# smacke/ffsubsync

Measured on AMD Instinct MI355X. Metric: alignments/sec (2 h@100 Hz, 7 framerate ratios), higher is better.
Workload: dtype i32; 1 GPU; configs[2]: 8192 x 7200 s@100 Hz pairs per GPU (8 batches of 1024), MaxScoreAligner over 7 framerate ratios, max_offset_samples=6000; algorithm=auto, pairs_per_gpu=8192, pairs_in_flight=512, n_fft_reference=2097152, n_fft_device=786432, input_format=bit-packed 0/1 vectors (FFS_DTYPE_U1) resident in HBM, parallelism=single GPU

## Files before the change

ffsubsync_amd/csrc/ffs_runs.h:

```cpp
#pragma once
#include "ffs_kernels.h"

namespace ffsa {

#ifndef FFS_RUNS_THREADS
#define FFS_RUNS_THREADS 512
#define FFS_RUNS_T 12288
#define FFS_RUNS_QCAP 3070
#endif
constexpr int RUNS_THREADS = FFS_RUNS_THREADS;
constexpr int RUNS_WAVES = RUNS_THREADS / 64;
constexpr int RUNS_T = FFS_RUNS_T;
constexpr int RUNS_LPT = RUNS_T / RUNS_THREADS;
constexpr int RUNS_QCAP = FFS_RUNS_QCAP;
static_assert(RUNS_T % RUNS_THREADS == 0 && RUNS_LPT % 4 == 0 && RUNS_LPT <= 32, "whole groups of four lags per thread, 32-bit edge windows");
constexpr int RUNS_CAP = 32768;
#ifndef FFS_RUNS_TPW
#define FFS_RUNS_TPW 2
#endif
constexpr int RUNS_TPW = FFS_RUNS_TPW;
constexpr int RUNS_QSENT = 0x1fffffff;
static_assert(RUNS_LPT <= 32 && RUNS_LPT % 4 == 0 && RUNS_QCAP % 2 == 0, "one 32-bit mask per thread, 8-byte histogram loads");

struct RunsRef {
// ... 67 lines not shown
}

FFS_DEV float wave_max_f32(float v) {
#define FFS_DPP_MAX(ctrl, rows) v = fmaxf(v, __int_as_float(__builtin_amdgcn_update_dpp(__float_as_int(v), __float_as_int(v), ctrl, rows, 0xf, false)))
    FFS_DPP_MAX(0x111, 0xf);
    FFS_DPP_MAX(0x112, 0xf);
    FFS_DPP_MAX(0x114, 0xf);
    FFS_DPP_MAX(0x118, 0xf);
    FFS_DPP_MAX(0x142, 0xa);
    FFS_DPP_MAX(0x143, 0xc);
#undef FFS_DPP_MAX
    return __int_as_float(__builtin_amdgcn_readlane(__float_as_int(v), 63));
}

constexpr int RUNS_XQ = 256;
template <int NT>
FFS_DEV void runs_extract_lds(unsigned (*&s_e)[NT / 64 * 2], unsigned (*&s_o)[NT / 64 * 2], uint4 (*&s_q)[RUNS_XQ]) {
    __shared__ unsigned l_e[2][NT / 64 * 2], l_o[2][NT / 64 * 2];
    __shared__ __attribute__((aligned(16))) uint4 l_q[NT / 64][RUNS_XQ];
    s_e = l_e, s_o = l_o, s_q = l_q;
}
template <int NT, bool compact = false>
FFS_DEV void runs_extract_body(const unsigned* __restrict__ w_generic, const int len, int2* __restrict__ e, int2* __restrict__ hdr,
                               const int cap) {
    constexpr int NWV = NT / 64;
    constexpr int G = 2, SWEEP = NT * 4 * G;
    const int tid = threadIdx.x, lane = tid & 63, wave = __builtin_amdgcn_readfirstlane(tid >> 6);
    const gptr eb = (gptr)e;
    const int nw = (len + 31) >> 5;
    const int n_proc = (len >> 5) + 1;
    const unsigned tail = (len & 31) ? ((1u << (len & 31)) - 1u) : 0xffffffffu;
    unsigned(*s_e)[NWV * 2], (*s_o)[NWV * 2];
    uint4(*s_q)[RUNS_XQ];
    runs_extract_lds<NT>(s_e, s_o, s_q);
    uint4* const ring = s_q[wave];
    unsigned q_head = 0, q_tail = 0;
    unsigned n_bound = 0, n_ones = 0;
    unsigned xn[G][4], pn[G];
    const __amdgpu_buffer_rsrc_t vrs = __builtin_amdgcn_make_buffer_rsrc(const_cast<unsigned*>(w_generic), 0, nw * 4, 0x00020000);
    auto request = [&](int base) {
#pragma unroll
        for (int g = 0; g < G; ++g) {
            const int w0 = base + (g * NT + tid) * 4;
            typedef unsigned v4u __attribute__((ext_vector_type(4)));
            const v4u t = __builtin_amdgcn_raw_buffer_load_b128(vrs, w0 * 4, 0, 2);
            xn[g][0] = t.x, xn[g][1] = t.y, xn[g][2] = t.z, xn[g][3] = t.w;
            pn[g] = 0;
            if (lane == 0) pn[g] = __builtin_amdgcn_raw_buffer_load_b32(vrs, w0 * 4 - 4, 0, 0);
        }
    };
// ... 162 lines not shown
        long long est = (long long)cnt * (long long)r.len / sampled;
        if (est > 0x3fffffff) est = 0x3fffffff;
        const_cast<int2*>(r.hdr)[0] = make_int2((int)est, 0);
    }
}

FFS_DEV void runs_extract_zero(int* __restrict__ zero, int zero_words) {
    if (zero && blockIdx.x == 0)
        for (int i = threadIdx.x; i < zero_words; i += blockDim.x) zero[i] = 0;
}
FFS_DEV bool runs_compact_vec(int cstride, int n_plain) {
    return cstride > 0 && (int)blockIdx.x < n_plain && (int)blockIdx.x % cstride != 0;
}
__global__ __launch_bounds__(256, 8) void k_runs_extract(const RunsRef* __restrict__ refs, int* __restrict__ zero, int zero_words,
                                                         int cstride, int n_plain) {
    runs_extract_zero(zero, zero_words);
    const RunsRef r = refs[blockIdx.x];
    if (!r.bits) return;
    if (runs_compact_vec(cstride, n_plain))
        runs_extract_body<256, true>(r.bits, r.len, const_cast<int2*>(r.e), const_cast<int2*>(r.hdr), r.cap);
    else
        runs_extract_body<256, false>(r.bits, r.len, const_cast<int2*>(r.e), const_cast<int2*>(r.hdr), r.cap);
}
__global__ __launch_bounds__(512, 4) void k_runs_extract_512(const RunsRef* __restrict__ refs, int with_len_cap, int* __restrict__ zero,
                                                             int zero_words, int cstride, int n_plain) {
    runs_extract_zero(zero, zero_words);
    const RunsRef r = refs[blockIdx.x];
    if (!r.bits) return;
    if (with_len_cap && threadIdx.x == 0) const_cast<int2*>(r.hdr)[1] = make_int2(r.len, r.cap);
    if (runs_compact_vec(cstride, n_plain))
        runs_extract_body<512, true>(r.bits, r.len, const_cast<int2*>(r.e), const_cast<int2*>(r.hdr), r.cap);
    else
        runs_extract_body<512, false>(r.bits, r.len, const_cast<int2*>(r.e), const_cast<int2*>(r.hdr), r.cap);
}
__global__ __launch_bounds__(1024, 4) void k_runs_extract_1024(const RunsRef* __restrict__ refs, int with_len_cap, int* __restrict__ zero,
                                                               int zero_words, int cstride, int n_plain) {
    runs_extract_zero(zero, zero_words);
    const RunsRef r = refs[blockIdx.x];
    if (!r.bits) return;
    if (with_len_cap && threadIdx.x == 0) const_cast<int2*>(r.hdr)[1] = make_int2(r.len, r.cap);
    if (runs_compact_vec(cstride, n_plain))
        runs_extract_body<1024, true>(r.bits, r.len, const_cast<int2*>(r.e), const_cast<int2*>(r.hdr), r.cap);
    else
        runs_extract_body<1024, false>(r.bits, r.len, const_cast<int2*>(r.e), const_cast<int2*>(r.hdr), r.cap);
}

__global__ __launch_bounds__(256, 8) void k_runs_extract_lists(const RunsRef* __restrict__ refs) {
    const RunsRef r = refs[blockIdx.x];
    if (threadIdx.x == 0) const_cast<int2*>(r.hdr)[1] = make_int2(r.len, r.cap);
    runs_extract_body<256>(r.bits, r.len, const_cast<int2*>(r.e), const_cast<int2*>(r.hdr), r.cap);
}

__global__ __launch_bounds__(1024, 4) void k_runs_extract_one(const unsigned* __restrict__ bits, int len, int2* __restrict__ e,
                                                             int2* __restrict__ hdr, int cap) {
    if (threadIdx.x == 0) hdr[1] = make_int2(len, cap);
    runs_extract_body<1024>(bits, len, e, hdr, cap);
}

static inline void runs_extract_launch(const RunsRef* refs, size_t n_vec, bool with_len_cap, hipStream_t st, int* zero = nullptr,
                                       int zero_words = 0, int cstride = 0, int n_plain = 0) {
    if (with_len_cap) cstride = 0;
    if (n_vec <= 256)
        hipLaunchKernelGGL(k_runs_extract_1024, dim3((unsigned)n_vec), dim3(1024), 0, st, refs, with_len_cap ? 1 : 0, zero, zero_words, cstride, n_plain);
    else if (n_vec <= 768)
        hipLaunchKernelGGL(k_runs_extract_512, dim3((unsigned)n_vec), dim3(512), 0, st, refs, with_len_cap ? 1 : 0, zero, zero_words, cstride, n_plain);
    else if (with_len_cap)
        hipLaunchKernelGGL(k_runs_extract_lists, dim3((unsigned)n_vec), dim3(256), 0, st, refs);
    else
        hipLaunchKernelGGL(k_runs_extract, dim3((unsigned)n_vec), dim3(256), 0, st, refs, zero, zero_words, cstride, n_plain);
}

FFS_DEV unsigned fetch32(GWords w, int len, long long start) {
    const int nw = (len + 31) >> 5;
    const long long wi = start >> 5;
    unsigned v[2];
#pragma unroll
    for (int k = 0; k < 2; ++k) {
        const long long i = wi + k;
        unsigned t = (i >= 0 && i < nw) ? w[i] : 0u;
        if (i == nw - 1 && (len & 31)) t &= (1u << (len & 31)) - 1u;
        v[k] = t;
    }
    return __builtin_amdgcn_alignbit(v[1], v[0], (unsigned)(start & 31));
}

FFS_DEV unsigned list_bits32(GEntries e, int n, long long start) {
    if (start + 32 <= 0 || n <= 0) return 0u;
    int lo = 0, hi = n;
    while (lo < hi) {
        const int mid = (lo + hi) >> 1;
        if ((long long)e[mid].pos <= start)
            lo = mid + 1;
// ... 1100 lines not shown
```

ffsubsync_amd/csrc/ffsalign.hip:

```cpp
#include <hip/hip_runtime.h>
#if defined(__x86_64__) && !defined(__HIP_DEVICE_COMPILE__)
#include <immintrin.h>
#define FFS_HOST_AVX2 1
#else
#define FFS_HOST_AVX2 0
#endif
#include <dlfcn.h>
#include <math.h>
#include <stdarg.h>
#include <stdio.h>
#include <stdlib.h>
#include <string.h>

#include <algorithm>
#include <chrono>
#include <string>
#include <mutex>
#include <vector>

#include "../../include/ffsubsync_amd.h"
#include "ffs_kernels.h"
#include "ffs_runs.h"
#include "ffs_split.h"
#include "ffs_quality.h"
// ... 52 lines not shown
            constexpr int DT = 4;                 \
            stmt;                                 \
        } else if ((dtype) == FFS_DTYPE_U8) {     \
            constexpr int DT = 0;                 \
            stmt;                                 \
        } else if ((dtype) == FFS_DTYPE_F32) {    \
            constexpr int DT = 1;                 \
            stmt;                                 \
        } else if ((dtype) == FFS_DTYPE_F64) {    \
            constexpr int DT = 3;                 \
            stmt;                                 \
        } else {                                  \
            constexpr int DT = 2;                 \
            stmt;                                 \
        }                                         \
    } while (0)

constexpr int64_t kMinFftN = 4096;
constexpr int64_t kMaxFftN = 1 << 24;
constexpr unsigned kPoolCapacity = 1u << 20;
constexpr long long kRunsBudgetPerPoint = 12;
constexpr int kRunsStride0 = 4096;
constexpr size_t kSmallCallCands = 4096;
constexpr int kSegBlocks = 3;
constexpr int kCollectRows = 4;

int ilog2(int64_t x) {
    int p = 0;
    while ((int64_t(1) << p) < x) ++p;
    return p;
}

int tile_cols(int L) {
    if (L % 3 == 0) {
        const int c = 3072 / L;
        return c < 16 ? 16 : c;
    }
    if (L <= 16) return 256;
    if (L <= 128) return 4096 / L;
    if (L <= 1024) return 16;
    if (L == 2048) return 8;
    return 4;
}

size_t col_lds_bytes(int L) {
    size_t t = (L > 16) ? (size_t)L * tile_cols(L) * sizeof(cf) : 0;
// ... 81 lines not shown
    int64_t workspace_bytes = 0;
    bool radix3_off = false;
    bool workspace_ready = false;
    int algo = FFS_ALGO_AUTO;
    int runs_split = 0;
    long long runs_budget = -1;
    int2* runs_e = nullptr;
    int runs_stride = 4096;
    size_t runs_e_entries = 0;
    int2* runs_n = nullptr;
    size_t runs_vecs = 0;
    unsigned* pack_buf = nullptr;
    size_t pack_bytes = 0;
    int* runs_flags = nullptr;
    int* runs_zero_flags = nullptr;
    int* runs_flags_host = nullptr;
    size_t runs_flags_n = 0;
    RunsBest* runs_best = nullptr;
    size_t runs_best_n = 0;
    bool runs_prev_fft = false;
    unsigned* lvl_buf = nullptr;
    size_t lvl_bytes = 0;
    hipEvent_t runs_ev = nullptr;
    int64_t runs_calls = 0, runs_fft_chunks = 0, runs_chunks = 0, runs_last_boundaries = 0;
    bool host_timing = false;
    double ht_vec = 0, ht_cand = 0, ht_wait = 0, ht_decide = 0, ht_total = 0;
    mutable std::vector<const void*> lds_configured;
    bool profiling = false;
    std::vector<hipEvent_t> ev_pool;
    size_t ev_used = 0;
    std::vector<std::pair<int, std::pair<hipEvent_t, hipEvent_t>>> ev_spans;
};

namespace {

template <class T>
int upload(T** dst, const std::vector<T>& src, int64_t* total) {
    HIP_TRY(hipMalloc((void**)dst, src.size() * sizeof(T)));
    HIP_TRY(hipMemcpy(*dst, src.data(), src.size() * sizeof(T), hipMemcpyHostToDevice));
    *total += (int64_t)(src.size() * sizeof(T));
    return FFS_OK;
}

int ensure_desc(ffs_plan* p, size_t bytes) {
    if (bytes <= p->dev_desc_bytes) return FFS_OK;
    if (p->upload_done) HIP_TRY(hipEventSynchronize(p->upload_done));
// ... 17 lines not shown
    static hipStream_t streams[64] = {};
    if (device < 0 || device >= 64) return nullptr;
    std::lock_guard<std::mutex> lock(mu);
    if (!streams[device] && hipStreamCreateWithFlags(&streams[device], hipStreamNonBlocking) != hipSuccess) {
        (void)hipGetLastError();
        streams[device] = nullptr;
    }
    return streams[device];
}
bool ensure_copy(ffs_plan* p) {
    if (!p->copy_stream) {
        p->copy_stream = shared_copy_stream(p->device);
        if (!p->copy_stream) return false;
    }
    if (!p->copy_ev && hipEventCreateWithFlags(&p->copy_ev, hipEventDisableTiming) != hipSuccess) {
        (void)hipGetLastError();
        p->copy_ev = nullptr;
        return false;
    }
    if (!p->dev_desc2 && hipMalloc(&p->dev_desc2, p->dev_desc_bytes) != hipSuccess) {
        (void)hipGetLastError();
        p->dev_desc2 = nullptr;
        return false;
    }
    return true;
}

int ensure_lds(const ffs_plan* p, const void* fn, size_t bytes) {
    for (const void* f : p->lds_configured)
        if (f == fn) return FFS_OK;
    HIP_TRY(hipFuncSetAttribute(fn, hipFuncAttributeMaxDynamicSharedMemorySize, (int)bytes));
    p->lds_configured.push_back(fn);
    return FFS_OK;
}

int ensure_workspace(ffs_plan* p) {
    if (p->direct_only || p->workspace_ready) return FFS_OK;
    const size_t work_bytes = (size_t)p->pairs_in_flight * p->max_slots * p->N * sizeof(cf);
    const size_t bn_bytes = (size_t)p->pairs_in_flight * (p->max_slots - 1) * 2 * (p->N2 / p->C) * sizeof(BlockNom);
    bool ok = hipMalloc((void**)&p->work, work_bytes) == hipSuccess;
    ok = ok && hipMalloc((void**)&p->bnom, bn_bytes) == hipSuccess;
    ok = ok && hipMalloc((void**)&p->xlist, (1 + (size_t)p->pairs_in_flight * p->max_cand) * sizeof(int)) == hipSuccess;
    ok = ok && hipMalloc((void**)&p->pool_entries, (size_t)kPoolCapacity * sizeof(PoolEntry)) == hipSuccess;
    int rc = FFS_OK;
    if (!ok) {
        (void)hipGetLastError();
// ... 662 lines not shown
    HIP_TRY(hipEventCreateWithFlags(&p->upload_done, hipEventDisableTiming));
    HIP_TRY(hipEventCreateWithFlags(&p->last_done, hipEventDisableTiming));
    for (int h = 0; h < 2; ++h) HIP_TRY(hipEventCreateWithFlags(&p->half_done[h], hipEventDisableTiming));
    {
        auto on = [](const char* name) {
            const char* e = getenv(name);
            return e && e[0] == '1';
        };
        p->allow_pruned = !on("FFS_DISABLE_PRUNED_PASS_C");
        p->allow_seg = !on("FFS_DISABLE_SEGMENTED");
        p->allow_half_last = !on("FFS_DISABLE_HALF_LAST");
        if (const char* ea = getenv("FFS_ALGORITHM")) {
            if (!strcmp(ea, "fft")) p->algo = FFS_ALGO_FFT;
            else if (!strcmp(ea, "runs")) p->algo = FFS_ALGO_RUNS;
        }
        p->runs_budget = -1;
        if (const char* eb = getenv("FFS_RUNS_BUDGET")) p->runs_budget = atoll(eb);
        if (const char* es = getenv("FFS_RUNS_SPLIT")) p->runs_split = atoi(es);
        p->runs_stride = kRunsStride0;
        if (const char* es = getenv("FFS_RUNS_STRIDE")) {
            const int v = atoi(es);
            p->runs_stride = v < 64 ? 64 : (v > RUNS_CAP ? RUNS_CAP : v);
        }
        if (const char* et = getenv("FFS_HOST_TIMING")) p->host_timing = et[0] == '1';
        const char* e3 = getenv("FFS_PASS_A_PREFETCH");
        if (e3) p->pass_a_prefetch = p->pass_a_prefetch_bits = atoi(e3);
#ifdef FFS_LAB
        const char* e20 = getenv("FFS_PASS_A_DEBUG");
        if (e20) p->lab_flags |= (atoi(e20) & 31) << 10;
        const char* e15 = getenv("FFS_MID_DEBUG");
        if (e15) p->lab_flags |= ((atoi(e15) & 1) ? DBG_NO_FFT : 0) | ((atoi(e15) & 2) ? DBG_HOT_MEM : 0) | ((atoi(e15) & 4) ? DBG_NO_STORE : 0);
#endif
    }
    if (n_fft < kMinFftN) {
        p->direct_only = true;
        guard.p = nullptr;
        *out = p;
        return FFS_OK;
    }
    if (r3) {
        p->N2 = n_fft >= 48 * 4096 ? 4096 : (int)(n_fft / 48);
        p->N1 = (int)(n_fft / p->N2);
    } else {
        const int lg = ilog2(n_fft);
        const int lg2 = lg - 4 < 12 ? lg - 4 : 12;
        p->N2 = 1 << lg2;
// ... 82 lines not shown
    (void)hipFree(p->tbA);
    (void)hipFree(p->tsA);
    (void)hipFree(p->tw1h);
    (void)hipFree(p->tbR);
    (void)hipFree(p->tsR);
    (void)hipFree(p->thR);
    (void)hipFree(p->tbM);
    (void)hipFree(p->tsM);
    (void)hipFree(p->twn1);
    (void)hipFree(p->work);
    (void)hipFree(p->bnom);
    (void)hipFree(p->pool_entries);
    (void)hipFree(p->xlist);
    if (p->seg) (void)ffs_plan_destroy(p->seg);
    (void)hipFree(p->runs_e);
    (void)hipFree(p->runs_n);
    (void)hipFree(p->runs_best);
    (void)hipFree(p->runs_flags);
    (void)hipFree(p->runs_zero_flags);
    (void)hipFree(p->pack_buf);
    (void)hipFree(p->lvl_buf);
    if (p->runs_flags_host) (void)hipHostFree(p->runs_flags_host);
    if (p->runs_ev) (void)hipEventDestroy(p->runs_ev);
    if (p->upload_done) (void)hipEventSynchronize(p->upload_done);
    if (p->copy_ev) (void)hipEventDestroy(p->copy_ev);
    for (int h = 0; h < 2; ++h)
        if (p->half_done[h]) (void)hipEventDestroy(p->half_done[h]);
    (void)hipFree(p->dev_desc);
    (void)hipFree(p->dev_desc2);
    if (p->host_desc) (void)hipHostFree(p->host_desc);
    if (p->upload_done) (void)hipEventDestroy(p->upload_done);
    if (p->last_done) (void)hipEventDestroy(p->last_done);
    for (hipEvent_t e : p->ev_pool) (void)hipEventDestroy(e);
    delete p;
    return FFS_OK;
}

int64_t ffs_plan_workspace_bytes(const ffs_plan* p) { return p ? p->workspace_bytes : 0; }

}

namespace {

struct AlignArgs {
    int n_pairs, n_cand, ref_dt, dtype;
    const void* const* vec_ptr;
// ... 183 lines not shown
    int32_t* level_lens(char* b) const { return (int32_t*)(b + o_ml); }
    int32_t* level_words(char* b) const { return (int32_t*)(b + o_mw); }
    XformDesc* xforms(char* b) const { return (XformDesc*)(b + o_xf); }
    NomList* nominees(char* b) const { return (NomList*)(b + o_nom); }
    RescoreAcc* acc(char* b) const { return (RescoreAcc*)(b + o_acc); }
    PoolBest* pool_best(char* b) const { return (PoolBest*)(b + o_pbest); }
    size_t table_at() const { return o_rv; }
    size_t table_bytes(size_t n_refs) const { return n_refs * sizeof(RunsRef); }
    size_t level_tables_bytes() const { return o_xf - o_rv; }
    size_t head_bytes(size_t n_refs) const { return o_rv + n_refs * sizeof(RunsRef); }
    size_t transform_bytes(size_t n_xf) const { return o_xf + n_xf * sizeof(XformDesc); }
    size_t refresh_at() const { return o_cand; }
    size_t refresh_bytes(size_t n_xf) const { return transform_bytes(n_xf) - o_cand; }
    size_t acc_bytes(size_t n) const { return n * KNOM * sizeof(RescoreAcc); }
    size_t acc_and_best_bytes() const { return acc_bytes(n_cands) + n_cands * sizeof(PoolBest); }
};

struct StreamLeave {
    ffs_plan* p;
    hipStream_t st;
    bool armed = false;
    bool upload_open = false;
    hipStream_t upload_st = nullptr;
    ~StreamLeave() {
        if (upload_open) (void)hipEventRecord(p->upload_done, upload_st);
        if (armed) (void)leave_stream(p, st);
    }
};

struct AlignCall {
    ffs_plan* const p;
    const AlignArgs& a;
    const hipStream_t st;
    StreamLeave leave;
    const int n_pairs, n_cand, stride, n_packed, n_slots, n_chunks;
    const size_t n_vec, n_cands;
    size_t n_rr = 0;
    size_t flag_bytes = 0;
    bool lists_in, ml, runs_ok, need_extract, ml_on = false, mixed, use_copy = false, dense_stream = false;
    int t_dtype, t_ref_dt;
    int hflags = 0;
    long long budget = 0;
    DescLayout L;
    char *hb = nullptr, *db = nullptr;
    CandDesc* hc = nullptr;
    const CandDesc* dc = nullptr;
    const RunsRef* d_rv = nullptr;
    const XformDesc* dx = nullptr;
    NomList* dn = nullptr;
    RescoreAcc* da = nullptr;
    PoolBest* dpb = nullptr;
    PoolArgs pa{};
    CandResult* cres;
    PairResult* pres;
    bool late_extract = false;
    bool probe_first = false;
    bool flags_cleared = false;
    bool copy_entered = false;
    bool proven = false, xf_built = false, retry = false;
    int tiles_max = 1;
    int64_t lvl_len_max = 1;
    const void* const* xptr;
    std::vector<const void*> expanded;
    BinList bins;
    bool pruned = false, seg = false;
    int seg_blocks = 0;
    int64_t seg_lo = 0;
    size_t n_xf;
    std::vector<char> chunk_fft;
    bool any_fft = false;
    double ht0 = 0, ht1 = 0, ht2 = 0, ht3 = 0;

    AlignCall(ffs_plan* p_, const AlignArgs& a_)
        : p(p_), a(a_), st((hipStream_t)a_.hip_stream), leave{p_, (hipStream_t)a_.hip_stream},
          n_pairs(a_.n_pairs), n_cand(a_.n_cand), stride(1 + a_.n_cand), n_packed((a_.n_cand + 1) / 2), n_slots(1 + (a_.n_cand + 1) / 2),
          n_chunks((a_.n_pairs + p_->pairs_in_flight - 1) / p_->pairs_in_flight), n_vec((size_t)a_.n_pairs * (1 + a_.n_cand)),
          n_cands((size_t)a_.n_pairs * a_.n_cand), cres((CandResult*)a_.cand_out_dev), pres((PairResult*)a_.pair_out_dev),
          xptr(a_.vec_ptr), n_xf((size_t)a_.n_pairs * (1 + (a_.n_cand + 1) / 2)) {
        memset(&bins, 0, sizeof bins);
        const bool may_run = p->algo != FFS_ALGO_FFT && !p->direct_only;
        lists_in = a.dtype == FFS_DTYPE_RUNS || a.ref_dt == FFS_DTYPE_RUNS;
        ml = may_run && (a.ref_dt == FFS_DTYPE_F64 || a.ref_dt == FFS_DTYPE_F32) && runs_able(a.dtype);
// ... 22 lines not shown
        if (on_copy && !copy_entered) {
            if (p->half_used[p->cur_half]) HIP_TRY(hipStreamWaitEvent(us, p->half_done[p->cur_half], 0));
            copy_entered = true;
        }
        HIP_TRY(hipMemcpyAsync(db + off, hb + off, bytes, hipMemcpyHostToDevice, us));
        leave.armed = true;
        leave.upload_open = true;
        leave.upload_st = us;
        const hipEvent_t ev = table_ahead ? p->copy_ev : p->upload_done;
        if (!table_ahead || on_copy) HIP_TRY(hipEventRecord(ev, us));
        if (on_copy) HIP_TRY(hipStreamWaitEvent(st, ev, 0));
        if (!table_ahead) leave.upload_open = false;
        return FFS_OK;
    }
    void launch_extraction(size_t n_refs, bool clear_flags, bool plain_lists) {
        ProfSpan span(p, st, FFS_K_RUNS_EXTRACT);
        if (plain_lists)
            runs_extract_launch(d_rv, n_refs, false, st, clear_flags ? p->runs_flags : nullptr, clear_flags ? (int)(flag_bytes / sizeof(int)) : 0,
                                stride, (int)n_vec);
        else
            runs_extract_launch(d_rv, n_refs, false, st, p->runs_flags, (int)(flag_bytes / sizeof(int)));
        flags_cleared = flags_cleared || clear_flags;
    }

    int prepare() {
        int rc;
        if (runs_ok && (rc = ensure_runs(p, need_extract ? n_rr : 0, 0, (size_t)n_chunks))) {
            if (lists_in || p->algo != FFS_ALGO_AUTO) return rc;
            runs_ok = false;
        }
        ml_on = runs_ok && ml;
        L = DescLayout((size_t)n_pairs, (size_t)n_cand, n_rr, ml_on, runs_ok,
                       p->seg ? (size_t)n_pairs * kSegBlocks * n_slots : n_xf);
        if ((rc = ensure_desc(p, L.total))) return rc;
        HIP_TRY(hipEventSynchronize(p->upload_done));
        hb = (char*)p->host_desc;
        memset(L.pool(hb), 0, 64);
        L.pool(hb)->capacity = kPoolCapacity;
        dense_stream = p->algo == FFS_ALGO_AUTO && p->runs_prev_fft && !lists_in;
        use_copy = runs_ok && need_extract && !ml_on && !dense_stream && ensure_copy(p);
        p->cur_half = use_copy ? 1 - p->cur_half : 0;
        db = (char*)(p->cur_half ? p->dev_desc2 : p->dev_desc);
        hc = L.cands(hb);
        dc = L.cands(db);
        d_rv = L.runs_refs(db);
        dx = L.xforms(db);
        dn = L.nominees(db);
        da = L.acc(db);
        dpb = L.pool_best(db);
        pa = PoolArgs{dn, L.pool(db), nullptr, dpb, n_chunks};
        pa.half_last = (hflags & HALF_LAST) ? 1 : 0;
        chunk_fft.assign((size_t)n_chunks, runs_ok ? 0 : 1);
        any_fft = !runs_ok;
        return FFS_OK;
    }
    int fill_runs_table() {
        RunsRef* hrv = L.runs_refs(hb);
        for (size_t i = 0; i < n_vec; ++i) {
            const int dt = (i % stride) ? a.dtype : a.ref_dt;
            if (dt == FFS_DTYPE_RUNS)
                hrv[i] = RunsRef{(const int2*)((const char*)a.vec_ptr[i] + 16), (const int2*)a.vec_ptr[i], nullptr, (int32_t)a.vec_len[i], 0};
            else if (dt == FFS_DTYPE_U1)
                hrv[i] = RunsRef{p->runs_e + i * (size_t)p->runs_stride, p->runs_n + i, (const unsigned*)a.vec_ptr[i], (int32_t)a.vec_len[i], p->runs_stride};
// ... 21 lines not shown
        return FFS_OK;
    }
    template <class T>
    void launch_levels() {
        const unsigned chunks = (unsigned)((lvl_len_max + 16383) / 16384);
        LevelInfo* d_li = L.level_info(db);
        hipLaunchKernelGGL((k_levels_sample<T>), dim3((unsigned)n_pairs), dim3(256), 0, st, (const T* const*)L.level_samples(db),
                           (const int*)L.level_lens(db), d_li);
        hipLaunchKernelGGL((k_levels_bits<T>), dim3(chunks, (unsigned)n_pairs), dim3(256), 0, st, (const T* const*)L.level_samples(db),
                           (const int*)L.level_lens(db), d_li, (unsigned* const*)L.level_planes(db), (const int*)L.level_words(db));
    }
    int start_extraction_early() {
        int rc;
        if (ml_on) {
            if ((rc = upload(L.table_at(), L.level_tables_bytes(), false, true))) return rc;
            {
                ProfSpan lspan(p, st, FFS_K_LEVELS);
                if (a.ref_dt == FFS_DTYPE_F64) launch_levels<double>();
                else launch_levels<float>();
            }
            HIP_TRY(hipGetLastError());
            launch_extraction(n_rr, true, false);
            HIP_TRY(hipGetLastError());
        } else if (need_extract && n_cands <= kSmallCallCands && !dense_stream) {
            late_extract = true;
        } else if (need_extract) {
            if ((rc = upload(L.table_at(), L.table_bytes(n_vec), use_copy, true))) return rc;
            probe_first = dense_stream;
            if (probe_first)
                hipLaunchKernelGGL(k_runs_probe, dim3((unsigned)((n_vec + 3) / 4)), dim3(256), 0, st, d_rv, (int)n_vec);
            else
                launch_extraction(n_vec, true, true);
            HIP_TRY(hipGetLastError());
        }
        return FFS_OK;
    }
    int fill_all_cands(const void* const* ptrs) {
        for (int pi = 0; pi < n_pairs; ++pi) {
            const size_t b = (size_t)pi * stride;
            const VecView ref = view(ptrs, b);
            for (int j = 0; j < n_cand; ++j) {
                CandDesc& cd = hc[(size_t)pi * n_cand + j];
                int rc;
                if ((rc = fill_cand(p, ref, view(ptrs, b + 1 + j), a.max_offset_samples, &cd, t_ref_dt, t_dtype))) return rc;
                if (runs_ok && !(cd.flags & CAND_NO_LAGS)) {
                    const int t = (cd.d_hi - cd.d_lo + RUNS_T) / RUNS_T;
                    if (t > tiles_max) tiles_max = t;
                }
            }
        }
        return FFS_OK;
    }
    int build_xforms() {
        int rc;
// ... 93 lines not shown
        if ((rc = upload(0, runs_ok ? L.head_bytes(with_table ? n_rr : 0) : L.transform_bytes(n_xf), use_copy))) return rc;
        if (late_extract) {
            launch_extraction(n_vec, true, true);
            HIP_TRY(hipGetLastError());
        }
        return FFS_OK;
    }
    int run_direct() {
        FFS_BY_RESCORE_DTYPE(mixed, t_dtype, hipLaunchKernelGGL((k_direct<DT>), dim3((unsigned)n_cands), dim3(256), 0, st, dc, cres));
        HIP_TRY(hipGetLastError());
        hipLaunchKernelGGL(k_finalize_pairs, dim3((n_pairs + 255) / 256), dim3(256), 0, st, cres, pres, n_pairs, n_cand,
                           (long long)a.filter_max_offset);
        HIP_TRY(hipGetLastError());
        return FFS_OK;
    }

    unsigned long long* d_stats() const { return (unsigned long long*)((char*)p->runs_flags + flag_bytes - 16); }
    void launch_chunk_flags(int from_estimates) {
        hipLaunchKernelGGL(k_runs_chunk_flags, dim3((unsigned)n_chunks, runs_flag_split((long long)p->pairs_in_flight * n_cand)), dim3(256), 0, st,
                           dc, n_pairs, n_cand, p->pairs_in_flight, d_rv, budget, p->runs_flags, d_stats(), from_estimates);
    }
    int read_flags_async() {
        HIP_TRY(hipGetLastError());
        HIP_TRY(hipMemcpyAsync(p->runs_flags_host, p->runs_flags, flag_bytes, hipMemcpyDeviceToHost, st));
        HIP_TRY(hipEventRecord(p->runs_ev, st));
        return FFS_OK;
    }
    int run_boundary_path() {
        int rc;
        if ((rc = ensure_runs(p, need_extract ? n_rr : 0, tiles_max > 1 ? n_cands * (size_t)tiles_max : 0, (size_t)n_chunks))) return rc;
        proven = bounds_prove_budget();
        bool skip_runs = false;
        if (probe_first && (rc = probe_dense_stream(&skip_runs))) return rc;
        if (skip_runs) return transforms_only();
        if ((rc = launch_flags_and_corr())) return rc;
        mark(&ht2);
        p->runs_calls += 1;
        p->runs_chunks += n_chunks;
        p->runs_last_boundaries = -1;
        return proven ? FFS_OK : read_back_and_decide();
    }
    bool bounds_prove_budget() const {
        if (need_extract || !a.vec_bound) return false;
        for (int pi = 0; pi < n_pairs; ++pi) {
            const size_t bq = (size_t)pi * stride;
            if (a.vec_bound[bq] <= 0) return false;
            for (int j = 0; j < n_cand; ++j) {
                const CandDesc& cd = hc[(size_t)pi * n_cand + j];
                if (a.vec_bound[bq + 1 + j] <= 0 ||
                    (!(cd.flags & CAND_NO_LAGS) &&
                     runs_over_budget(a.vec_bound[bq + 1 + j], a.vec_bound[bq], RUNS_CAP, RUNS_CAP, (long long)cd.d_hi - cd.d_lo + 1, cd.R, budget)))
                    return false;
            }
        }
        return true;
    }
    int probe_dense_stream(bool* skip_runs) {
        int rc;
// ... 31 lines not shown
                launch_chunk_flags(0);
            if ((rc = read_flags_async())) return rc;
        }
        {
            ProfSpan span(p, st, FFS_K_RUNS_CORR);
            if (ml_on) {
                hipLaunchKernelGGL(k_runs_corr_ml, dim3((unsigned)n_cands, (unsigned)tiles_max), dim3(RUNS_THREADS), 0, st, dc, n_cand, d_rv,
                                   cres, p->runs_best, tiles_max, d_flags, p->pairs_in_flight, (const LevelInfo*)L.level_info(db), (int)n_vec);
            } else {
                int split = n_cand;
                if (p->runs_split > 0) split = p->runs_split < n_cand ? p->runs_split : n_cand;
                hipLaunchKernelGGL(k_runs_corr, dim3((unsigned)((size_t)n_pairs * split), (unsigned)tiles_max), dim3(RUNS_THREADS), 0, st, dc,
                                   n_cand, d_rv, cres, p->runs_best, tiles_max, d_flags, p->pairs_in_flight, split);
            }
            if (tiles_max > 1)
                hipLaunchKernelGGL(k_runs_pick, dim3((unsigned)((n_cands + 255) / 256)), dim3(256), 0, st, dc, (int)n_cands, n_cand,
                                   p->runs_best, tiles_max, cres, d_flags, p->pairs_in_flight);
        }
        hipLaunchKernelGGL(k_finalize_pairs, dim3((n_pairs + 255) / 256), dim3(256), 0, st, cres, pres, n_pairs, n_cand,
                           (long long)a.filter_max_offset);
        HIP_TRY(hipGetLastError());
        return FFS_OK;
    }
    int read_back_and_decide() {
        int rc;
        if (!xf_built && p->runs_prev_fft && !lists_in && (rc = build_xforms())) return rc;
        HIP_TRY(hipEventSynchronize(p->runs_ev));
        mark(&ht3);
        bool bad = false;
        for (int ch = 0; ch < n_chunks; ++ch) {
            const int f = p->runs_flags_host[ch];
            if (f == 2) bad = true;
            if (f) chunk_fft[ch] = 1, any_fft = true;
        }
        memcpy(&p->runs_last_boundaries, (char*)p->runs_flags_host + flag_bytes - 16, 8);
        long long longest = 0;
        memcpy(&longest, (char*)p->runs_flags_host + flag_bytes - 8, 8);
        if (need_extract && longest >= p->runs_stride && p->runs_stride < RUNS_CAP) {
            p->runs_stride = p->runs_stride * 4 < RUNS_CAP ? p->runs_stride * 4 : RUNS_CAP;
            p->runs_calls -= 1;
            p->runs_chunks -= n_chunks;
            retry = true;
            return FFS_OK;
        }
        if (bad)
            return fail(FFS_E_INVALID, "a boundary list of the call is truncated (more entries than its block holds): "
                        "nothing can solve it -- pass the vector as bits");
        p->runs_prev_fft = any_fft;
        return any_fft ? upload_for_fallback() : FFS_OK;
    }
// ... 87 lines not shown
        }
        FFS_BY_RESCORE_DTYPE(mixed, t_dtype, hipLaunchKernelGGL((k_pool_rescore<DT>), dim3(2048), dim3(256), 0, st, dc, pa.header, pa.entries, dpb));
        hipLaunchKernelGGL(k_pool_pick, dim3(256), dim3(256), 0, st, pa.header, pa.entries, dpb);
        return FFS_OK;
    }
    void finalize_range(size_t c0, size_t c1, int p0, int p1) {
        hipLaunchKernelGGL(k_finalize_cands, dim3((unsigned)((c1 - c0 + 255) / 256)), dim3(256), 0, st, dc + c0, dn + c0, da + c0 * KNOM,
                           cres + c0, (int)(c1 - c0), mixed ? 4 : t_dtype, pa.header, dpb + c0);
        hipLaunchKernelGGL(k_finalize_pairs, dim3((unsigned)((p1 - p0 + 255) / 256)), dim3(256), 0, st, cres + (size_t)p0 * n_cand, pres + p0,
                           p1 - p0, n_cand, (long long)a.filter_max_offset);
    }
    int finalize_transformed() {
        if (!runs_ok) finalize_range(0, n_cands, 0, n_pairs);
        for (int ch = 0; runs_ok && ch < n_chunks; ++ch) {
            if (!chunk_fft[ch]) continue;
            const int p0 = ch * p->pairs_in_flight, p1 = (p0 + p->pairs_in_flight) < n_pairs ? (p0 + p->pairs_in_flight) : n_pairs;
            finalize_range((size_t)p0 * n_cand, (size_t)p1 * n_cand, p0, p1);
        }
        HIP_TRY(hipGetLastError());
        return FFS_OK;
    }
    int finish() {
        leave.armed = false;
        const int rc = leave_stream(p, st);
        if (p->host_timing && runs_ok && !retry) {
            const double ht4 = now_ns();
            p->ht_vec += ht1 - ht0, p->ht_cand += ht2 - ht1, p->ht_wait += ht3 - ht2, p->ht_decide += ht4 - ht3, p->ht_total += ht4 - ht0;
        }
        return rc;
    }
};

int solve_call(ffs_plan* p, const AlignArgs& a, bool* retry) {
    static_assert(sizeof(CandResult) == sizeof(ffs_cand_result), "ABI struct mismatch");
    static_assert(sizeof(PairResult) == sizeof(ffs_pair_result), "ABI struct mismatch");
    *retry = false;
    HIP_TRY(hipSetDevice(p->device));
    int rc;
    AlignCall c(p, a);
    if ((rc = enter_stream(p, c.st))) return rc;
    c.ht0 = c.ht1 = c.ht2 = c.ht3 = p->host_timing ? now_ns() : 0.0;
    if ((rc = c.prepare())) return rc;
    if (c.runs_ok) {
        if ((rc = c.fill_runs_table())) return rc;
        if ((rc = c.start_extraction_early())) return rc;
    }
// ... 2378 lines not shown
```

Before: 2.690 million 7-ratio solves/s.

## Pipeline run extraction on a priority stream overlapping per-part correlation

Splits the batch of pairs into parts and runs run-list extraction plus chunk flags for each part on a separate high-priority stream. Correlation of part k on the main stream waits only on that part's event, so extraction of later parts can overlap with correlation of earlier ones. Later parts use a new persistent grid-strided extraction kernel with a capped grid so it leaves compute units free for the concurrent correlation. This adds event and stream synchronization complexity and more kernel launches, and the per-part flag and correlation launches are smaller.

```diff
diff --git a/ffsubsync_amd/csrc/ffs_runs.h b/ffsubsync_amd/csrc/ffs_runs.h
--- a/ffsubsync_amd/csrc/ffs_runs.h
+++ b/ffsubsync_amd/csrc/ffs_runs.h
@@ -113,10 +113,10 @@
 }
 template <int NT, bool compact = false>
 FFS_DEV void runs_extract_body(const unsigned* __restrict__ w_generic, const int len, int2* __restrict__ e, int2* __restrict__ hdr,
-                               const int cap) {
+                               const int cap, const int tid_in = (int)threadIdx.x) {
     constexpr int NWV = NT / 64;
     constexpr int G = 2, SWEEP = NT * 4 * G;
-    const int tid = threadIdx.x, lane = tid & 63, wave = __builtin_amdgcn_readfirstlane(tid >> 6);
+    const int tid = tid_in, lane = tid & 63, wave = __builtin_amdgcn_readfirstlane(tid >> 6);
     const gptr eb = (gptr)e;
     const int nw = (len + 31) >> 5;
     const int n_proc = (len >> 5) + 1;
@@ -325,6 +325,23 @@
     else
         runs_extract_body<256, false>(r.bits, r.len, const_cast<int2*>(r.e), const_cast<int2*>(r.hdr), r.cap);
 }
+__global__ __launch_bounds__(256, 8) void k_runs_extract_walk(const RunsRef* __restrict__ refs, int n_pairs) {
+    const RunsRef* rp = refs + blockIdx.y;
+    const int wave_s = __builtin_amdgcn_readfirstlane((int)threadIdx.x >> 6);
+    for (int pair = (int)blockIdx.x; pair < n_pairs; pair += (int)gridDim.x) {
+        const RunsRef r = rp[(size_t)pair * gridDim.y];
+        int ones = -1;
+        asm volatile("" : "+s"(ones));
+        const int tid = wave_s * 64 + (int)__builtin_amdgcn_mbcnt_hi((unsigned)ones, __builtin_amdgcn_mbcnt_lo((unsigned)ones, 0u));
+        if (r.bits) {
+            if (blockIdx.y != 0)
+                runs_extract_body<256, true>(r.bits, r.len, const_cast<int2*>(r.e), const_cast<int2*>(r.hdr), r.cap, tid);
+            else
+                runs_extract_body<256, false>(r.bits, r.len, const_cast<int2*>(r.e), const_cast<int2*>(r.hdr), r.cap, tid);
+        }
+        __syncthreads();
+    }
+}
 __global__ __launch_bounds__(512, 4) void k_runs_extract_512(const RunsRef* __restrict__ refs, int with_len_cap, int* __restrict__ zero,
                                                              int zero_words, int cstride, int n_plain) {
     runs_extract_zero(zero, zero_words);
@@ -371,6 +388,11 @@
         hipLaunchKernelGGL(k_runs_extract_lists, dim3((unsigned)n_vec), dim3(256), 0, st, refs);
     else
         hipLaunchKernelGGL(k_runs_extract, dim3((unsigned)n_vec), dim3(256), 0, st, refs, zero, zero_words, cstride, n_plain);
+}
+static inline void runs_extract_launch_walk(const RunsRef* refs, int n_pairs, int stride, int grid, hipStream_t st) {
+    int gx = (grid + stride - 1) / stride;
+    gx = gx < n_pairs ? gx : n_pairs;
+    hipLaunchKernelGGL(k_runs_extract_walk, dim3((unsigned)gx, (unsigned)stride), dim3(256), 0, st, refs, n_pairs);
 }
 
 FFS_DEV unsigned fetch32(GWords w, int len, long long start) {
diff --git a/ffsubsync_amd/csrc/ffsalign.hip b/ffsubsync_amd/csrc/ffsalign.hip
--- a/ffsubsync_amd/csrc/ffsalign.hip
+++ b/ffsubsync_amd/csrc/ffsalign.hip
@@ -98,6 +98,7 @@
 constexpr long long kRunsBudgetPerPoint = 12;
 constexpr int kRunsStride0 = 4096;
 constexpr size_t kSmallCallCands = 4096;
+constexpr int kPipeParts = 8, kPipeMinPairs = 2048, kPipeGrid = 512, kPipePartsMax = 64;
 constexpr int kSegBlocks = 3;
 constexpr int kCollectRows = 4;
 
@@ -225,6 +226,11 @@
     unsigned* lvl_buf = nullptr;
     size_t lvl_bytes = 0;
     hipEvent_t runs_ev = nullptr;
+    int pipe_parts = kPipeParts;
+    int pipe_min_pairs = kPipeMinPairs;
+    int pipe_grid = kPipeGrid;
+    hipStream_t extract_stream = nullptr;
+    std::vector<hipEvent_t> part_ev;
     int64_t runs_calls = 0, runs_fft_chunks = 0, runs_chunks = 0, runs_last_boundaries = 0;
     bool host_timing = false;
     double ht_vec = 0, ht_cand = 0, ht_wait = 0, ht_decide = 0, ht_total = 0;
@@ -288,6 +294,37 @@
         (void)hipGetLastError();
         p->dev_desc2 = nullptr;
         return false;
+    }
+    return true;
+}
+
+hipStream_t shared_extract_stream(int device) {
+    static std::mutex mu;
+    static hipStream_t streams[64] = {};
+    if (device < 0 || device >= 64) return nullptr;
+    std::lock_guard<std::mutex> lock(mu);
+    if (!streams[device]) {
+        int least = 0, greatest = 0;
+        if (hipDeviceGetStreamPriorityRange(&least, &greatest) != hipSuccess ||
+            hipStreamCreateWithPriority(&streams[device], hipStreamNonBlocking, greatest) != hipSuccess) {
+            (void)hipGetLastError();
+            streams[device] = nullptr;
+        }
+    }
+    return streams[device];
+}
+bool ensure_parts(ffs_plan* p, int parts) {
+    if (!p->extract_stream) {
+        p->extract_stream = shared_extract_stream(p->device);
+        if (!p->extract_stream) return false;
+    }
+    while ((int)p->part_ev.size() < parts) {
+        hipEvent_t e = nullptr;
+        if (hipEventCreateWithFlags(&e, hipEventDisableTiming) != hipSuccess) {
+            (void)hipGetLastError();
+            return false;
+        }
+        p->part_ev.push_back(e);
     }
     return true;
 }
@@ -996,6 +1033,13 @@
             const int v = atoi(es);
             p->runs_stride = v < 64 ? 64 : (v > RUNS_CAP ? RUNS_CAP : v);
         }
+        if (const char* ep = getenv("FFS_RUNS_PIPELINE")) {
+            int v[3] = {p->pipe_parts, p->pipe_min_pairs, p->pipe_grid};
+            const int n = sscanf(ep, "%d,%d,%d", &v[0], &v[1], &v[2]);
+            if (n >= 1) p->pipe_parts = v[0] < 0 ? 0 : (v[0] > kPipePartsMax ? kPipePartsMax : v[0]);
+            if (n >= 2) p->pipe_min_pairs = v[1] < 0 ? 0 : v[1];
+            if (n >= 3) p->pipe_grid = v[2] < 0 ? 0 : v[2];
+        }
         if (const char* et = getenv("FFS_HOST_TIMING")) p->host_timing = et[0] == '1';
         const char* e3 = getenv("FFS_PASS_A_PREFETCH");
         if (e3) p->pass_a_prefetch = p->pass_a_prefetch_bits = atoi(e3);
@@ -1124,6 +1168,7 @@
     (void)hipFree(p->lvl_buf);
     if (p->runs_flags_host) (void)hipHostFree(p->runs_flags_host);
     if (p->runs_ev) (void)hipEventDestroy(p->runs_ev);
+    for (hipEvent_t e : p->part_ev) (void)hipEventDestroy(e);
     if (p->upload_done) (void)hipEventSynchronize(p->upload_done);
     if (p->copy_ev) (void)hipEventDestroy(p->copy_ev);
     for (int h = 0; h < 2; ++h)
@@ -1353,8 +1398,10 @@
     bool armed = false;
     bool upload_open = false;
     hipStream_t upload_st = nullptr;
+    hipEvent_t x_last = nullptr;
     ~StreamLeave() {
         if (upload_open) (void)hipEventRecord(p->upload_done, upload_st);
+        if (x_last) (void)hipStreamWaitEvent(st, x_last, 0);
         if (armed) (void)leave_stream(p, st);
     }
 };
@@ -1389,6 +1436,9 @@
     bool flags_cleared = false;
     bool copy_entered = false;
     bool proven = false, xf_built = false, retry = false;
+    bool piped = false;
+    int n_parts = 1, part_chunks = 0;
+    hipStream_t xs = nullptr;
     int tiles_max = 1;
     int64_t lvl_len_max = 1;
     const void* const* xptr;
@@ -1457,6 +1507,33 @@
             runs_extract_launch(d_rv, n_refs, false, st, p->runs_flags, (int)(flag_bytes / sizeof(int)));
         flags_cleared = flags_cleared || clear_flags;
     }
+    int part_pair0(int k) const { return k * part_chunks * p->pairs_in_flight; }
+    int part_pairs(int k) const {
+        const int p0 = part_pair0(k), np = part_chunks * p->pairs_in_flight;
+        return (n_pairs - p0) < np ? (n_pairs - p0) : np;
+    }
+    int record_on_xs(hipEvent_t ev) {
+        HIP_TRY(hipEventRecord(ev, xs));
+        leave.x_last = ev;
+        return FFS_OK;
+    }
+    int enter_extract_stream() {
+        HIP_TRY(hipStreamWaitEvent(xs, p->copy_ev, 0));
+        if (p->has_last) HIP_TRY(hipStreamWaitEvent(xs, p->last_done, 0));
+        return FFS_OK;
+    }
+    void launch_extraction_part(int k) {
+        ProfSpan span(p, xs, FFS_K_RUNS_EXTRACT);
+        const RunsRef* rv = d_rv + (size_t)part_pair0(k) * stride;
+        const size_t nv = (size_t)part_pairs(k) * stride;
+        if (k == 0)
+            runs_extract_launch(rv, nv, false, xs, p->runs_flags, (int)(flag_bytes / sizeof(int)), stride, (int)nv);
+        else if (p->pipe_grid > 0)
+            runs_extract_launch_walk(rv, part_pairs(k), stride, p->pipe_grid, xs);
+        else
+            runs_extract_launch(rv, nv, false, xs, nullptr, 0, stride, (int)nv);
+        flags_cleared = true;
+    }
 
     int prepare() {
         int rc;
@@ -1474,6 +1551,13 @@
         L.pool(hb)->capacity = kPoolCapacity;
         dense_stream = p->algo == FFS_ALGO_AUTO && p->runs_prev_fft && !lists_in;
         use_copy = runs_ok && need_extract && !ml_on && !dense_stream && ensure_copy(p);
+        if (use_copy && !lists_in && p->pipe_parts > 1 && n_pairs >= p->pipe_min_pairs && n_chunks > 1) {
+            part_chunks = (n_chunks + p->pipe_parts - 1) / p->pipe_parts;
+            n_parts = (n_chunks + part_chunks - 1) / part_chunks;
+            piped = n_parts > 1 && ensure_parts(p, n_parts);
+            if (piped) xs = p->extract_stream;
+            else n_parts = 1;
+        }
         p->cur_half = use_copy ? 1 - p->cur_half : 0;
         db = (char*)(p->cur_half ? p->dev_desc2 : p->dev_desc);
         hc = L.cands(hb);
@@ -1541,14 +1625,18 @@
             HIP_TRY(hipGetLastError());
             launch_extraction(n_rr, true, false);
             HIP_TRY(hipGetLastError());
-        } else if (need_extract && n_cands <= kSmallCallCands && !dense_stream) {
+        } else if (need_extract && n_cands <= kSmallCallCands && !dense_stream && !piped) {
             late_extract = true;
         } else if (need_extract) {
             if ((rc = upload(L.table_at(), L.table_bytes(n_vec), use_copy, true))) return rc;
             probe_first = dense_stream;
             if (probe_first)
                 hipLaunchKernelGGL(k_runs_probe, dim3((unsigned)((n_vec + 3) / 4)), dim3(256), 0, st, d_rv, (int)n_vec);
-            else
+            else if (piped) {
+                if ((rc = enter_extract_stream())) return rc;
+                launch_extraction_part(0);
+                if ((rc = record_on_xs(p->part_ev[0]))) return rc;
+            } else
                 launch_extraction(n_vec, true, true);
             HIP_TRY(hipGetLastError());
         }
@@ -1688,7 +1776,8 @@
     }
     int read_flags_async() {
         HIP_TRY(hipGetLastError());
-        HIP_TRY(hipMemcpyAsync(p->runs_flags_host, p->runs_flags, flag_bytes, hipMemcpyDeviceToHost, st));
+        HIP_TRY(hipMemcpyAsync(p->runs_flags_host, p->runs_flags, flag_bytes, hipMemcpyDeviceToHost, piped ? xs : st));
+        if (piped) return record_on_xs(p->runs_ev);
         HIP_TRY(hipEventRecord(p->runs_ev, st));
         return FFS_OK;
     }
@@ -1699,7 +1788,7 @@
         bool skip_runs = false;
         if (probe_first && (rc = probe_dense_stream(&skip_runs))) return rc;
         if (skip_runs) return transforms_only();
-        if ((rc = launch_flags_and_corr())) return rc;
+        if ((rc = piped ? launch_parts() : launch_flags_and_corr())) return rc;
         mark(&ht2);
         p->runs_calls += 1;
         p->runs_chunks += n_chunks;
@@ -1777,10 +1866,43 @@
         HIP_TRY(hipGetLastError());
         return FFS_OK;
     }
+    int launch_parts() {
+        int rc;
+        const int pif = p->pairs_in_flight;
+        HIP_TRY(hipStreamWaitEvent(xs, p->upload_done, 0));
+        int split = n_cand;
+        if (p->runs_split > 0) split = p->runs_split < n_cand ? p->runs_split : n_cand;
+        for (int k = 0; k < n_parts; ++k) {
+            const int p0 = part_pair0(k), np = part_pairs(k), ch0 = k * part_chunks, nch = (np + pif - 1) / pif;
+            const size_t c0 = (size_t)p0 * n_cand, nc = (size_t)np * n_cand;
+            const CandDesc* dck = dc + c0;
+            const RunsRef* rvk = d_rv + (size_t)p0 * stride;
+            const int* flk = p->runs_flags + ch0;
+            RunsBest* bestk = p->runs_best ? p->runs_best + c0 * (size_t)tiles_max : nullptr;
+            if (k) launch_extraction_part(k);
+            hipLaunchKernelGGL(k_runs_chunk_flags, dim3((unsigned)nch, runs_flag_split((long long)pif * n_cand)), dim3(256), 0, xs, dck, np, n_cand,
+                               pif, rvk, budget, p->runs_flags + ch0, d_stats(), 0);
+            HIP_TRY(hipGetLastError());
+            if ((rc = record_on_xs(p->part_ev[k]))) return rc;
+            HIP_TRY(hipStreamWaitEvent(st, p->part_ev[k], 0));
+            ProfSpan span(p, st, FFS_K_RUNS_CORR);
+            hipLaunchKernelGGL(k_runs_corr, dim3((unsigned)((size_t)np * split), (unsigned)tiles_max), dim3(RUNS_THREADS), 0, st, dck, n_cand,
+                               rvk, cres + c0, bestk, tiles_max, flk, pif, split);
+            if (tiles_max > 1)
+                hipLaunchKernelGGL(k_runs_pick, dim3((unsigned)((nc + 255) / 256)), dim3(256), 0, st, dck, (int)nc, n_cand, bestk, tiles_max,
+                                   cres + c0, flk, pif);
+        }
+        if ((rc = read_flags_async())) return rc;
+        hipLaunchKernelGGL(k_finalize_pairs, dim3((n_pairs + 255) / 256), dim3(256), 0, st, cres, pres, n_pairs, n_cand,
+                           (long long)a.filter_max_offset);
+        HIP_TRY(hipGetLastError());
+        return FFS_OK;
+    }
     int read_back_and_decide() {
         int rc;
         if (!xf_built && p->runs_prev_fft && !lists_in && (rc = build_xforms())) return rc;
         HIP_TRY(hipEventSynchronize(p->runs_ev));
+        leave.x_last = nullptr;
         mark(&ht3);
         bool bad = false;
         for (int ch = 0; ch < n_chunks; ++ch) {
@@ -1914,6 +2036,10 @@
     }
     int finish() {
         leave.armed = false;
+        if (leave.x_last) {
+            HIP_TRY(hipStreamWaitEvent(st, leave.x_last, 0));
+            leave.x_last = nullptr;
+        }
         const int rc = leave_stream(p, st);
         if (p->host_timing && runs_ok && !retry) {
             const double ht4 = now_ns();
diff --git a/profiles/runs_pipeline_ab.py b/profiles/runs_pipeline_ab.py
--- /dev/null
+++ b/profiles/runs_pipeline_ab.py
@@ -0,0 +1,71 @@
+import json, os, sys, time
+ROOT = os.path.dirname(os.path.dirname(os.path.abspath(__file__)))
+sys.path.insert(0, ROOT)
+import numpy as np
+import torch
+from ffsubsync_amd import _native, batch
+from workloads import synth
+
+out_path = sys.argv[1]
+n = int(sys.argv[2]) if len(sys.argv) > 2 else 8192
+rounds = int(sys.argv[3]) if len(sys.argv) > 3 else 5
+steps = int(sys.argv[4]) if len(sys.argv) > 4 else 20
+variants = [("off", "0")] + [("k%d_g%d" % (k, g), "%d,1,%d" % (k, g)) for k in (4, 8, 16) for g in (0, 256, 512, 768, 1024)]
+
+specs = [synth.make_pair_spec(s) for s in range(n)]
+db = synth.build_device_batch(specs)
+n_fft = db.required_fft_length(6000)
+cand_out = torch.empty(n * 7 * 24, dtype=torch.uint8, device="cuda")
+pair_out = torch.empty(n * 24, dtype=torch.uint8, device="cuda")
+aligners = {}
+for name, value in variants:
+    os.environ["FFS_RUNS_PIPELINE"] = value
+    aligners[name] = batch.BatchAligner(n_fft, 7, 6000, pairs_in_flight=min(512, n), algorithm="auto")
+del os.environ["FFS_RUNS_PIPELINE"]
+
+records = {}
+runs = {name: [] for name, _ in variants}
+host = {name: [] for name, _ in variants}
+for r in range(rounds):
+    for name, _ in variants:
+        al = aligners[name]
+        for _ in range(3):
+            al.solve_async(db, 0, n, cand_out, pair_out)
+        torch.cuda.synchronize()
+        h = 0.0
+        t0 = time.perf_counter()
+        for _ in range(steps):
+            h0 = time.perf_counter()
+            al.solve_async(db, 0, n, cand_out, pair_out)
+            h += time.perf_counter() - h0
+        torch.cuda.synchronize()
+        runs[name].append(1e3 * (time.perf_counter() - t0) / steps)
+        host[name].append(1e3 * h / steps)
+        if r == 0:
+            records[name] = (cand_out.cpu().numpy().tobytes(), pair_out.cpu().numpy().tobytes())
+
+kernels = {}
+for name, _ in variants:
+    al = aligners[name]
+    al.plan.profile(True)
+    al.solve_async(db, 0, n, cand_out, pair_out)
+    torch.cuda.synchronize()
+    kernels[name] = {k: {"ms": round(v[0], 4), "launches": v[1]} for k, v in al.plan.profile_read().items() if v[1]}
+    al.plan.profile(False)
+
+result = {"pairs": n, "steps": steps, "rounds": rounds, "n_fft": n_fft,
+          "what": "ms per step of %d pairs x 7 ratios, wall clock over %d queued steps, variants alternating per round" % (n, steps),
+          "variants": {name: {"FFS_RUNS_PIPELINE": value, "ms_per_step": [round(x, 4) for x in runs[name]],
+                              "median_ms": round(float(np.median(runs[name])), 4),
+                              "host_ms_per_call": [round(x, 4) for x in host[name]],
+                              "records_equal_off": records[name] == records["off"], "profiled_step": kernels[name]}
+                       for name, value in variants}}
+with open(out_path, "w") as f:
+    json.dump(result, f, indent=1)
+for name, _ in variants:
+    v = result["variants"][name]
+    print(name, v["median_ms"], v["ms_per_step"], "host", v["host_ms_per_call"][-1], "equal", v["records_equal_off"])
+for name, _ in variants:
+    sys.stderr.write("[variant %s]\n" % name)
+    sys.stderr.flush()
+    aligners[name].close()
diff --git a/profiles/runs_pipeline_trace.py b/profiles/runs_pipeline_trace.py
--- /dev/null
+++ b/profiles/runs_pipeline_trace.py
@@ -0,0 +1,42 @@
+import csv, glob, json, os, sys
+
+rows = []
+for path in glob.glob(os.path.join(sys.argv[1], "**", "*kernel_trace.csv"), recursive=True):
+    with open(path, newline="") as f:
+        for r in csv.DictReader(f):
+            rows.append((r["Kernel_Name"], int(r["Start_Timestamp"]), int(r["End_Timestamp"])))
+ext = sorted((a, b) for n, a, b in rows if "k_runs_extract" in n)
+corr = sorted((a, b) for n, a, b in rows if "k_runs_corr" in n)
+
+
+def merged(iv):
+    out = []
+    for a, b in iv:
+        if out and a <= out[-1][1]:
+            out[-1][1] = max(out[-1][1], b)
+        else:
+            out.append([a, b])
+    return out
+
+
+def intersection(x, y):
+    i = j = 0
+    tot = 0
+    while i < len(x) and j < len(y):
+        lo, hi = max(x[i][0], y[j][0]), min(x[i][1], y[j][1])
+        if hi > lo:
+            tot += hi - lo
+        if x[i][1] < y[j][1]:
+            i += 1
+        else:
+            j += 1
+    return tot
+
+
+me, mc = merged(ext), merged(corr)
+both = intersection(me, mc)
+busy = sum(b - a for a, b in merged(sorted(ext + corr)))
+sum_e, sum_c = sum(b - a for a, b in ext), sum(b - a for a, b in corr)
+print(json.dumps({"extract_launches": len(ext), "corr_launches": len(corr), "extract_sum_ms": sum_e / 1e6, "corr_sum_ms": sum_c / 1e6,
+                  "both_running_ms": both / 1e6, "overlapped_fraction_of_extraction": both / max(1, sum(b - a for a, b in me)),
+                  "either_running_ms": busy / 1e6}))
```

After: 2.311 million 7-ratio solves/s. -14.1%, worse.
